# vdBerg93/cl-rrt

Hardware: AMD Instinct MI355X
Metric: nodes expanded/sec (200-obstacle scene) (higher is better)
Workload: dtype f64

## Files before the change

### cl-rrt_amd/clrrt/__init__.py

```python
import ctypes as C
import os

import numpy as np

from . import abi
from .abi import (CLRRT_COLLISION_OBB, CLRRT_COLLISION_OCC, CLRRT_COLLISION_STUB, CLRRT_MODE_BATCH,
                  CLRRT_MODE_EXACT, ROLL_NAMES)

PKG_DIR = os.path.dirname(os.path.dirname(os.path.abspath(__file__)))
LIB_PATH = os.environ.get("CLRRT_LIB") or os.path.join(PKG_DIR, "libclrrt.so")
HEADER_PATH = os.path.join(os.path.dirname(PKG_DIR), "include", "clrrt.h")

_lib = None
P = C.POINTER
EXCHANGE_FN = C.CFUNCTYPE(C.c_int32, C.c_void_p, P(abi.ExchangeIO))

_SIGS = {
    "clrrt_abi_version": (C.c_int, []),
    "clrrt_params_default": (C.c_int, [P(abi.Params), C.c_double, P(C.c_double), C.c_double]),
    "clrrt_rng_seed": (None, [P(abi.Rng), C.c_uint32]),
    "clrrt_rng_next": (C.c_int32, [P(abi.Rng)]),
    "clrrt_draw_samples": (C.c_int, [P(abi.Params), P(abi.Rng), C.c_int32, P(abi.Sample)]),
    "clrrt_create": (C.c_int, [P(abi.Params), P(abi.Capacity), C.c_int, P(C.c_void_p)]),
    "clrrt_destroy": (None, [C.c_void_p]),
# ... 574 lines not shown
    def iterations(self):
        n = C.c_int64()
        self._chk(self.L.clrrt_iteration_records(self.h, 0, 0, None, C.byref(n)), "iteration_records")
        arr = (abi.Iteration * max(1, n.value))()
        self._chk(self.L.clrrt_iteration_records(self.h, 0, n.value, arr, C.byref(n)), "iteration_records")
        return {f: np.array([getattr(arr[i], f) for i in range(n.value)], dtype=np.int64)
                for f, _ in abi.Iteration._fields_}

    def round_sizes(self):
        n = C.c_int64()
        self._chk(self.L.clrrt_round_sizes(self.h, None, 0, C.byref(n)), "round_sizes")
        out = np.zeros(max(1, n.value), dtype=np.int64)
        self._chk(self.L.clrrt_round_sizes(self.h, out.ctypes.data_as(P(C.c_int64)), n.value, C.byref(n)), "round_sizes")
        return out[:n.value]

    def walk_audit(self, samples):
        n = len(samples)
        arr = (abi.Sample * n)(*samples)
        out = np.zeros((n, 20), dtype=np.int32)
        self._chk(self.L.clrrt_walk_audit(self.h, arr, n, out.ctypes.data_as(P(C.c_int32))), "walk_audit")
        return out

    WALK_TILE_DTYPE = np.dtype([(f, np.float32) for f in ("pcx", "pcy", "pr", "rcx", "rcy", "rr", "thx", "thy", "thh",
                                                         "apx", "apy", "aph", "cemin", "aopt")] +
                               [("nonfinite", np.int32), ("eroot", np.float32)])
    WALK_FN_IN = {0: 3, 1: 3, 2: 21, 3: 2, 4: 2}
    WALK_FN_OUT = {0: 2, 1: 2, 2: 2, 3: 2, 4: 3}

    def walk_index(self, first=0, count=None, fused=False):
        if count is None:
# ... 57 lines not shown
```

### cl-rrt_amd/csrc/clrrt_capi.hip

```cpp
#include <hip/hip_runtime.h>
#include <math.h>

#include <algorithm>
#include <climits>
#include <array>
#include <chrono>
#include <cmath>
#include <cstdio>
#include <cstdlib>
#include <cstring>
#include <deque>
#include <functional>
#include <optional>
#include <string>
#include <vector>

#include "../../include/clrrt.h"
#include "clrrt_dev.hpp"
#include "clrrt_devmem_hip.hpp"
#include "clrrt_internal.hpp"

static const int kWalkMaxOver = 2048, kWalkMaxChunks = 64;

using namespace clrrt;
// ... 95 lines not shown
  Job* jobs = nullptr;
  int64_t* totals = nullptr;
  bool totals_zeroed = false;
  unsigned long long* work_ctr = nullptr;
  float* nn_seed = nullptr;
  double bbox[4] = {HUGE_VAL, HUGE_VAL, -HUGE_VAL, -HUGE_VAL};
  double* d_bbox = nullptr;
  double* h_bbox = nullptr;
  int64_t nnw_min_nodes = 8192;
  bool nnw_stateless = false;
  int nnw_bud_tiles = 3072, nnw_bud_ex = 4096, nnw_chunks = 16, nnw_max_over = 1024;
  bool nnw_max_over_set = false;
  bool nnw_bud_tiles_set = false;
  int nnw_half_max = 4096;
  int nnw_hscale = 50;
  int nnw_root_seed = 1;
  int nnw_root_k = 64;
  int nnw_root_scan = 16384;
  int nnw_index = 5;
  int nnw_waves = -1;
  int nnw_double = 1;
  WalkBufs nnw{};
  WalkBufs nnw_alt{};
  BuiltFor nnw_built;
  CompactBufs cmp{};
  int roll_persistent = 1;
  int nn_debug = 0;
  int roll_blocks = 0;
  int n_cu = 256;
  int* roll_q = nullptr;
// ... 1480 lines not shown
    else if (k == "nn_root_k") c->nnw_root_k = (int)value;
    else c->nnw_root_scan = (int)value;
    c->nnw_built.n = -1;
  }
  else if (k == "nn_walk_index" && value >= 0 && value <= 5) {
    c->nnw_index = (int)value;
    c->nnw_built.n = -1;
    c->nnw.sorted_n = c->nnw_alt.sorted_n = c->nnw3.sorted_n = -1;
  }
  else if (k == "nn_walk_waves" && value >= -1 && value <= 1 << 20) c->nnw_waves = (int)value;
  else if (k == "nn_walk_chunks" && value >= 1 && value <= kWalkMaxChunks) c->nnw_chunks = (int)value;
  else if (k == "nn_walk_max_over" && value >= 1 && value <= kWalkMaxOver) {
    c->nnw_max_over = (int)value;
    c->nnw_max_over_set = true;
  }
  else if (k == "nn_walk_double") c->nnw_double = value != 0;
  else if (k == "nn_lag" && (value == 0 || value == 1 || value == 2)) c->nn_lag = (int)value;
  else if (k == "nn_delta_walk") c->nn_delta_walk = value != 0 ? 1 : 0;
  else if (k == "nn_delta_verify") c->nn_delta_verify = value != 0 ? 1 : 0;
  else if (k == "nn_debug" && value >= 0) c->nn_debug = (int)value;
  else if (k == "fail_at_round" && value >= 0 && value < INT_MAX) c->fail_at_round = (int)value;
  else if (k == "fail_after_exchange" && value >= 0 && value < INT_MAX) c->fail_after_exchange = (int)value;
  else if (k == "fail_in_round" && value >= 0 && value < INT_MAX) c->fail_in_round = (int)value;
  else if (k == "shard_hook_world1") c->sh.hook_world1 = value != 0;
  else if (k == "roll_blocks" && value >= 0 && value < (1 << 20)) c->roll_blocks = (int)value;
  else if (k == "nn_pipeline") c->nn_pipeline = value != 0;
  else if (k == "roll_priority") c->roll_priority = value != 0;
  else if (k == "roll_order_verify") c->roll_order_verify = value != 0;
  else if (k == "roll_coop") c->roll_coop = value != 0;
  else if (k == "roll_spread") c->roll_spread = value != 0;
// ... 69 lines not shown
  const int64_t Mp = c->cap.max_nodes + 1024;
  HIPC(c, c->mem.renew(&w.sorder, c->cap.max_batch));
  HIPC(c, c->mem.renew(&w.keys, 2 * M));
  HIPC(c, c->mem.renew(&w.keys2, 2 * M));
  HIPC(c, c->mem.renew(&w.vals, std::max<int64_t>(M, Mp)));
  HIPC(c, c->mem.renew(&w.vals2, M));
  w.tmp_bytes = walk_sort_bytes((int)M);
  HIPC(c, c->mem.renew_bytes(&w.tmp, std::max<size_t>(w.tmp_bytes, 256)));
  HIPC(c, c->mem.renew(&w.Q, Mp));
  HIPC(c, c->mem.renew(&w.CE, Mp));
  HIPC(c, c->mem.renew(&w.ID, Mp));
  HIPC(c, c->mem.renew(&w.HEAD, Mp));
  HIPC(c, c->mem.renew(&w.trun, walk_tile_count(c->cap.max_nodes) + 1));
  HIPC(c, c->mem.renew(&w.tiles, walk_tile_count(c->cap.max_nodes) + 1));
  HIPC(c, c->mem.renew(&w.supers, walk_super_count(c->cap.max_nodes) + 1));
  HIPC(c, c->mem.renew(&w.ovf_n, 1));
  HIPC(c, c->mem.renew(&w.ovf, kWalkMaxOver));
  HIPC(c, c->mem.renew(&w.wctr, 8 + 2 + 64));
  w.roster = w.wctr + 8;
  HIPC(c, c->mem.renew(&w.pk, (int64_t)kWalkMaxOver * kWalkMaxChunks * 11));
  HIPC(c, c->mem.renew(&w.pi, (int64_t)kWalkMaxOver * kWalkMaxChunks * 11));
  HIPC(c, c->mem.renew(&w.skeys, Mp));
  HIPC(c, c->mem.renew(&w.sids, Mp));
  w.sorted_n = -1;
  w.cap_nodes = c->cap.max_nodes;
  w.cap_batch = (int)c->cap.max_batch;
  HIPC(c, c->mem.renew(&w.P, Mp));
  return CLRRT_OK;
}

static int ensure_walk_set(clrrt_ctx* c, WalkBufs& w) {
  w.bud_tiles = c->nnw_bud_tiles_set || c->nnw_bud_tiles == 0
                    ? c->nnw_bud_tiles
                    : (int)std::max<int64_t>(c->nnw_bud_tiles, c->n_nodes >> 11);
  w.bud_ex = c->nnw_bud_ex > 0 ? (int)std::max<int64_t>(c->nnw_bud_ex, c->n_nodes >> 9) : 0;
  w.max_over = c->nnw_max_over_set || c->n_nodes < (6 << 20) ? c->nnw_max_over : kWalkMaxOver;
  w.nch = c->nnw_chunks;
  w.half_max = c->nnw_half_max;
  w.index_kind = c->nnw_index;
  w.hscale_pct = c->nnw_hscale;
  w.root_seed = c->nnw_root_seed;
  w.root_k = c->nnw_root_k;
  w.root_scan = c->nnw_root_scan;
  w.waves = c->nnw_waves < 0 ? 9 * c->n_cu : c->nnw_waves;
  w.waves_min_batch = c->nnw_waves < 0 ? 4 * w.waves : 0;
  return alloc_walk(c, w);
}
static int ensure_walk(clrrt_ctx* c) { return ensure_walk_set(c, c->nnw); }

static NnSetup nn_setup(clrrt_ctx* c) {
  NnSetup su;
  double& x0 = su.x0; double& y0 = su.y0; double& x1 = su.x1; double& y1 = su.y1;
  sample_region(c->params, x0, y0, x1, y1);
  if (c->bbox[0] <= c->bbox[2]) {
    x0 = std::min(x0, c->bbox[0] - 1.0); y0 = std::min(y0, c->bbox[1] - 1.0);
    x1 = std::max(x1, c->bbox[2] + 1.0); y1 = std::max(y1, c->bbox[3] + 1.0);
// ... 1850 lines not shown
  int rc = ensure_walk(c);
  if (rc != CLRRT_OK) return rc;
  memcpy(cur.h_samples, samples, sizeof(clrrt_sample) * n);
  HIPC(c, hipMemcpyAsync(cur.d_samples, cur.h_samples, sizeof(clrrt_sample) * n, hipMemcpyHostToDevice, c->stream));
  c->nnw_built.n = -1;
  HIPC(c, launch_nn_walk_build(c->stream, c->nn, (int)c->n_nodes, su.fr, su.x0, su.y0, su.x1, su.y1, c->nnw));
  const char* const pre = "clrrt_walk_audit: ";
  Scratch<int> d_out;
  HIPC(c, d_out.alloc(20 * (size_t)n));
  HIPP(c, pre, launch_walk_audit(c->stream, cur.d_samples, n, c->nn, (int)c->n_nodes, c->dp, su.fr, c->nnw, d_out));
  HIPP(c, pre, hipMemcpyAsync(out, d_out, sizeof(int32_t) * 20 * (size_t)n, hipMemcpyDeviceToHost, c->stream));
  HIPP(c, pre, hipStreamSynchronize(c->stream));
  return CLRRT_OK;
}

int clrrt_debug_walk_index(clrrt_ctx* c, int64_t first, int64_t count, int32_t fused, double hdr[9], float* P,
                           float* Q, float* CE, int32_t* ID, int32_t* HEAD, int32_t* trun, void* tiles, void* supers,
                           int32_t* roster) {
  if (!c || !hdr) return CLRRT_EINVAL;
  if (first < 0 || count <= 0 || first > c->n_nodes || count > c->n_nodes - first)
    return fail(c, CLRRT_EINVAL, "debug_walk_index: node range outside the tree");
  pf_reset(c);
  HIPC(c, hipSetDevice(c->device));
  const NnSetup su = nn_setup(c);
  const bool whole = !fused && first == 0 && count == c->n_nodes;
  if (!su.region_ok || c->n_nodes < c->nnw_min_nodes || (!fused && !whole && count < c->nnw_min_nodes))
    return fail(c, CLRRT_ESTATE, "the walk does not serve this tree (too small or no region)");
  int rc = CLRRT_OK;
  WalkBufs* w = nullptr;
  if (fused) {
// ... 63 lines not shown
```

### cl-rrt_amd/csrc/clrrt_internal.hpp

```cpp
#pragma once
#include <hip/hip_runtime.h>
#include <stdint.h>

#include "../../include/clrrt.h"
#include "clrrt_dev.hpp"
#include "clrrt_stdsort.hpp"

namespace clrrt {

#define CLRRT_ROLL_PENDING (-2)

struct RollRes {
  double st[10];
  double costE, costS;
  double bx, by;
  double fx, fy;
  double vback;
  int32_t outcome;
  int32_t nrows;
  int32_t refN;
  int32_t pad;
};

struct WorkCtr {
// ... 144 lines not shown
  int2* trun;
  WalkTile *tiles, *supers;
  int bud_tiles, bud_ex, max_over, nch;
  int half_max = 4096;
  int waves = 0;
  int waves_min_batch = 0;
  int index_kind = 0;
  int hscale_pct = 100;
  int* wctr = nullptr;
  int* roster = nullptr;
  int root_seed = 1;
  int root_k = 64;
  int root_scan = 16384;
  float* seed_out = nullptr;
  hipEvent_t ev_main = nullptr;
  int* ovf_n;
  int4* ovf;
  float* pk;
  int* pi;
  uint64_t* skeys;
  int* sids;
  int64_t sorted_n;
  double sorted_x0, sorted_y0, sorted_scale;
  int sorted_kind;
  int64_t cap_nodes;
  int cap_batch;
};
size_t walk_sort_bytes(int n);
int64_t walk_tile_count(int64_t n);
int64_t walk_super_count(int64_t n);
// ... 190 lines not shown
```

### cl-rrt_amd/csrc/clrrt_nnwalk.hip

```cpp
#include <hip/hip_runtime.h>
#include <climits>
#include <hip/hip_fp16.h>
#include <hipcub/hipcub.hpp>
#include <rocprim/device/device_merge.hpp>
#include <algorithm>
#include <stdint.h>

#include "clrrt_dev.hpp"
#include "clrrt_internal.hpp"

namespace clrrt {

#define CAND_K 10
#define NN_K (CAND_K + 1)
#define WALK_TILE 32
#define WALK_SUPER 32
#define WALK_FMT_STATE 0
#define WALK_FMT_HALF 1
#define WALK_FMT_CODED 2
#ifndef WALK_STAGE1_QUEUE
#define WALK_STAGE1_QUEUE 0
#endif
#ifndef WALK_HALF_SUPER
#define WALK_HALF_SUPER 1
// ... 93 lines not shown
    return;
  }
  uint32_t k = 0xffffffffu;
  if (isfinite(x) && isfinite(y)) {
    const double fx = fmin(fmax((x - x0) * scale, 0.0), 65535.0);
    const double fy = fmin(fmax((y - y0) * scale, 0.0), 65535.0);
    k = w_spread((uint32_t)fx) | (w_spread((uint32_t)fy) << 1);
  }
  keys[i] = ((uint64_t)bin << (64 - WALK_SECTOR_BITS)) | ((uint64_t)k << (32 - WALK_SECTOR_BITS)) |
            (__float_as_uint(nodes[i].costE) >> WALK_SECTOR_BITS);
  vals[i] = i;
}

__global__ void k_walk_skeys(const clrrt_sample* __restrict__ S, int B, double x0, double y0, double scale,
                             uint32_t* __restrict__ keys, int* __restrict__ vals, int* __restrict__ zero1,
                             int* __restrict__ zero8) {
  const int i = blockIdx.x * blockDim.x + threadIdx.x;
  if (zero1 && i == 0) *zero1 = 0;
  if (zero8 && i < 8) zero8[i] = 0;
  if (i >= B) return;
  const double x = S[i].x, y = S[i].y;
  uint32_t k = 0xffffffffu;
  if (isfinite(x) && isfinite(y)) {
    const double fx = fmin(fmax((x - x0) * scale, 0.0), 65535.0);
    const double fy = fmin(fmax((y - y0) * scale, 0.0), 65535.0);
    k = w_spread((uint32_t)fx) | (w_spread((uint32_t)fy) << 1);
  }
  keys[i] = k;
  vals[i] = i;
}

__global__ void k_walk_trun(const int* __restrict__ HEAD, const int* __restrict__ ID, int ntiles,
                            int2* __restrict__ trun) {
// ... 499 lines not shown
  float lim = __builtin_inff();
  float cb0 = -2.f;
  int n2 = 0;
#ifdef CLRRT_WALK_PROFILE
  const bool prof = fr.debug == 2;
#else
  constexpr bool prof = false;
#endif
  uint64_t cyc[4] = {0, 0, 0, 0};
#ifdef CLRRT_WALK_PROFILE
  unsigned long long hist[6] = {0, 0, 0, 0, 0, 0};
#endif
  int hc = -1;
  float kc = 0.f;
  __shared__ int s_root[4];
  int seeded = -1;
  if constexpr (!SPLIT) {
    float kr = -__builtin_inff();
    int rX = -1;
    if (roster && !ex) seeded = walk_root_seed(sx, sy, nodes, roster, p.feas_len, lane, kr, rX, lk, li);
    if (lane == 0) {
      s_root[0] = __float_as_int(kr);
      s_root[1] = rX;
      s_root[2] = seeded;
    }
    __builtin_amdgcn_wave_barrier();
  }
  unsigned long long n_sup = 0, n_tile = 0, n_q = 0, n_ex = 0, n_und = 0, n_sure = 0, n_drop = 0;

  auto refresh = [&]() __attribute__((always_inline)) {
    kth = uni(__shfl(lk, NN_K - 1, 64));
// ... 135 lines not shown
    const int cnt = __popcll(m);
    if (cnt == 0) return;
    if (n2 + cnt > 64) drain_exact(cnt);
    __builtin_amdgcn_wave_barrier();
    if (keep) {
      const int pos = n2 + __popcll(m & ((1ull << lane) - 1));
      s_q2[pos] = j;
      s_b2[pos] = lbt;
    }
    n2 += cnt;
    __builtin_amdgcn_wave_barrier();
  };
  auto drain = [&]() __attribute__((always_inline)) { drain_exact(64); };
  auto prefilter = [&](int id, int hd, float4 pp, float4 qq, float ce) __attribute__((always_inline)) -> bool {
    if (hd == hc && !w_less(kc, id, kth, idk)) return false;
    if constexpr (!SPLIT) {
      if (hd & WALK_ROOT_BIT) {
        if (id <= s_root[1] || !w_less(__int_as_float(s_root[0]), id, kth, idk)) return false;
      }
    }
    const float qx = rsx - pp.x, qy = rsy - pp.y;
    const float d2 = qx * qx + qy * qy;
    float l2 = lim;
    if (!ex) {
      const float R = (kth - ce + 2e-4f) * (1.0f / 0.9999f);
      l2 = R < 0.f ? -1.f : (R + dl) * (R + dl);
    }
    if (!(id >= 0 && ((d2 <= l2) || (l2 != l2)))) return false;
    const float vx = rsx - qq.x, vy = rsy - qq.y;
    const float dot = vx * qq.z + vy * qq.w, vv = vx * vx + vy * vy;
    const bool ang_bad = (vv < fl2) || (dot < -1e-3f) || (dot * dot < c45 * c45 * vv && dot >= 0.f);
// ... 66 lines not shown
    n_und += __popcll(__ballot(la == -__builtin_inff())) + __popcll(__ballot(lb == -__builtin_inff()));
    n_sure += __popcll(__ballot(ua < __builtin_inff())) + __popcll(__ballot(ub < __builtin_inff()));
    const bool ia = ub_insert(ua);
    const bool ib2 = ub_insert(ub);
    if (ia || ib2) refresh();
    enqueue(oka, la, ja);
    enqueue(okb, lb, jb);
#endif
    if (prof) cyc[2] += __builtin_amdgcn_s_memtime() - c0;
  };
  auto hmin = [&](float v) -> float {
#pragma unroll
    for (int o = 16; o > 0; o >>= 1) v = fminf(v, __shfl_xor(v, o, 64));
    return v;
  };
  auto run_out = [&](int tl) -> bool {
    const int2 tr = trun[tl];
    if constexpr (!SPLIT) {
      if (tr.x >= 0 && (tr.x & WALK_ROOT_BIT) && !w_less(__int_as_float(s_root[0]), tr.y, kth, idk)) return true;
    }
    return tr.x >= 0 && tr.x == hc && !w_less(kc, tr.y, kth, idk);
  };
  int qn = 0;
  auto next_q = [&]() __attribute__((always_inline)) -> int {
    while (qn > 0) {
      qn--;
      const int t = uni(s_tq[qn]);
      if (!(uni(s_tb[qn]) > kth)) return t;
    }
    return -1;
  };
  auto visit_queue = [&]() __attribute__((always_inline)) {
    const int t0 = next_q();
    const int t1 = next_q();
    const int t2 = next_q();
    const int t3 = next_q();
// ... 8 lines not shown
  };
  auto visit_supers = [&](int la, int lb2, float Tp, float T, bool first) {
    const uint64_t c0 = prof ? __builtin_amdgcn_s_memtime() : 0;
#if WALK_SPLIT_SHARE
    if constexpr (SPLIT && SHARE) refresh();
#endif
    n_sup += 1 + (lb2 >= 0);
    const int sa = gst(la), sb = lb2 >= 0 ? gst(lb2) : -1;
    const int lo = lane < 32 ? la : lb2;
    const int st = lane < 32 ? sa : sb;
    const int tl = st * WALK_SUPER + (lane & 31);
    float lb = __builtin_inff();
    uint64_t tm;
    if constexpr (STATE) {
      const uint32_t vis = st >= 0 ? s_vis[lo] : 0xffffffffu;
      if (st >= 0 && tl < ntiles && !((vis >> (lane & 31)) & 1u)) {
#if WALK_CHEAP_FIRST
        const WalkTile tt = tiles[tl];
        lb = walk_lb_dist(tt, rsx, rsy, ex, dsR);
        if (!(lb > fminf(T, kth))) lb = walk_lb(tt, rsx, rsy, ex, flen_t, dsR);
#else
        lb = walk_lb(tiles[tl], rsx, rsy, ex, flen_t, dsR);
#endif
        if (run_out(tl)) lb = __builtin_inff();
      }
      const bool take = st >= 0 && lb <= T && !(lb > kth);
      const bool drop = st >= 0 && lb > kth;
      tm = __ballot(take);
      const uint64_t dm = __ballot(drop);
      const float rest = hmin(take || drop || st < 0 ? __builtin_inff() : lb);
      if ((lane & 31) == 0 && st >= 0) {
        const int sh = lane;
        s_vis[lo] = vis | (uint32_t)(tm >> sh) | (uint32_t)(dm >> sh);
        s_lbf[lo] = rest;
      }
    } else {
      float slb;
      if constexpr (FMT == WALK_FMT_HALF && WALK_HALF_SUPER) {
        slb = st >= 0 ? __half2float(s_sh[lo]) : __builtin_inff();
// ... 30 lines not shown
    __builtin_amdgcn_wave_barrier();
    while (qn >= 4) visit_queue();
    if (prof) cyc[1] += __builtin_amdgcn_s_memtime() - c0;
  };

  const uint64_t ct0 = prof ? __builtin_amdgcn_s_memtime() : 0;
  auto flush_stats = [&]() {
    if (stats && lane == 0) {
      atomicAdd(&stats[0], n_sup);
      atomicAdd(&stats[1], n_tile);
      atomicAdd(&stats[2], n_q);
      atomicAdd(&stats[3], n_ex);
      atomicAdd(&stats[10], n_und);
      atomicAdd(&stats[11], n_sure);
      atomicAdd(&stats[12], n_drop);
      if (prof) {
        atomicAdd(&stats[4], (unsigned long long)cyc[0]);
        atomicAdd(&stats[5], (unsigned long long)cyc[1]);
        atomicAdd(&stats[6], (unsigned long long)cyc[2]);
        atomicAdd(&stats[7], (unsigned long long)cyc[3]);
        atomicAdd(&stats[8], (unsigned long long)(__builtin_amdgcn_s_memtime() - ct0));
#ifdef CLRRT_WALK_PROFILE
        atomicAdd(&stats[13], hist[0]);
        for (int q = 1; q < 6; q++) atomicAdd(&stats[14 + q], hist[q]);
#endif
      }
    }
  };
  if (SPLIT) refresh();
  if constexpr (!SPLIT) {
// ... 25 lines not shown
  __builtin_amdgcn_wave_barrier();
  if (prof) cyc[0] += __builtin_amdgcn_s_memtime() - ct0;
#ifndef WALK_T0
#define WALK_T0 0.5f
#endif
#ifndef WALK_GROW
#define WALK_GROW 2.f
#endif
  float T = base + WALK_T0, Tp = -__builtin_inff();
#if CLRRT_DELTA_ONEPASS
  if constexpr (SPLIT && !SHARE) {
    if (kb < __builtin_inff()) T = __builtin_inff();
  }
#endif
  bool budget = !SPLIT && (bud_tiles > 0 || bud_ex > 0);
  for (int pass = 0;; pass++) {
    const float lim_t = fminf(T, kth);
    const int lim_c = CODED ? uni(lc_le(lim_t - base)) : 0;
    for (int t0 = 0; t0 < nloc; t0 += 64) {
      const int t = t0 + lane;
      bool want;
      if constexpr (CODED) {
        const int c = t < nloc ? s_lb[t] : 255;
        want = c != 255 && c <= lim_c;
      } else {
        const float lb = t < nloc ? (STATE ? s_lbf[t] : __half2float(s_lbh[t])) : __builtin_inff();
        want = lb < __builtin_inff() && lb <= lim_t;
      }
      uint64_t m = __ballot(want);
      while (m) {
        int sa = -1, sb = -1;
        while (m && sb < 0) {
          const int st = t0 + __ffsll((unsigned long long)m) - 1;
          m &= m - 1;
          if (CODED ? (int)s_lb[st] > kth_c : (STATE ? s_lbf[st] : __half2float(s_lbh[st])) > kth) continue;
          if (sa < 0) sa = st; else sb = st;
        }
        if (sa >= 0) visit_supers(sa, sb, Tp, T, pass == 0);
        if (budget && ((bud_tiles > 0 && n_tile > (unsigned long long)bud_tiles) ||
                       (bud_ex > 0 && n_ex > (unsigned long long)bud_ex))) {
          int slot = 0;
          if (lane == 0) slot = atomicAdd(ovf_n, 1);
          slot = uni(__shfl(slot, 0, 64));
          if (slot < max_over) {
            if (lane == 0)
              ovf[slot] = make_int4(s, __float_as_int(kth), idk == 0x7fffffff ? idk : idk + 1,
                                    kth > 0.f ? __float_as_int(kth) : kth == 0.f ? 0 : 0x7f800000);
            if (stats && lane == 0) atomicAdd(&stats[14], 1ull);
            flush_stats();
            return;
          }
          budget = false;
        }
      }
    }
    flush_queue();
    drain();
    if (T == __builtin_inff() || kth <= T) break;
    Tp = T;
    T = base + (T - base) * WALK_GROW;
    if (T > 1e7f) T = __builtin_inff();
  }
  if constexpr (SPLIT) {
    const int o = o_sp;
    if (lane < NN_K) {
      pk[((size_t)o * nch + ch) * NN_K + lane] = lk;
      pi[((size_t)o * nch + ch) * NN_K + lane] = li;
    }
// ... 17 lines not shown
                                                    const WalkTile* __restrict__ tiles, int ntiles,
                                                    const WalkTile* __restrict__ sup, int nsup, DevParams p,
                                                    NnFrame fr, int* __restrict__ cand, float* __restrict__ ckey,
                                                    int* __restrict__ ncand, int* __restrict__ ctie,
                                                    const int* __restrict__ sorder,
                                                    unsigned long long* __restrict__ stats, int bud_tiles,
                                                    int bud_ex, int* __restrict__ ovf_n, int4* __restrict__ ovf,
                                                    int max_over, int nch, float* __restrict__ pk,
                                                    int* __restrict__ pi, int nloc_max, int* __restrict__ wctr,
                                                    const int* __restrict__ roster) {
  if constexpr (SPLIT) {
    const int o = (int)blockIdx.x / nch;
    const int ch = (int)blockIdx.x % nch;
    if (o >= min(*ovf_n, max_over)) return;
    const int4 rec = ovf[o];
    const int nloc = ch < nsup ? (nsup - ch + nch - 1) / nch : 0;
    walk_one<FMT, SPLIT, BRK>(S, B, nodes, P, Q, CE, ID, HEAD, trun, tiles, ntiles, sup, nsup, p, fr, cand, ckey, ncand, ctie, sorder, stats, bud_tiles, bud_ex, ovf_n, ovf, max_over, nch, pk, pi, nloc_max, rec.x, ch, nloc, __int_as_float(rec.y), rec.z, o);
  } else {
    const int per = (B + 7) >> 3;
    const int x0 = (int)(blockIdx.x & 7);
    if constexpr (!PERS) {
      const int t = x0 * per + (int)(blockIdx.x >> 3);
      if (t >= B) return;
      walk_one<FMT, SPLIT, BRK>(S, B, nodes, P, Q, CE, ID, HEAD, trun, tiles, ntiles, sup, nsup, p, fr, cand, ckey, ncand,
                                ctie, sorder, stats, bud_tiles, bud_ex, ovf_n, ovf, max_over, nch, pk, pi, nloc_max,
                                sorder[t], 0, nsup, __builtin_inff(), 0x7fffffff, 0, roster);
      return;
    }
    int k = 0;
    for (;;) {
      int t = -1;
      while (k < 8) {
        const int x = (x0 + k) & 7;
        int i = 0;
        if (threadIdx.x == 0) i = atomicAdd(&wctr[x], 1);
        i = __shfl(i, 0, 64);
        if (i < per && x * per + i < B) { t = x * per + i; break; }
        k++;
      }
      if (t < 0) break;
      walk_one<FMT, SPLIT, BRK>(S, B, nodes, P, Q, CE, ID, HEAD, trun, tiles, ntiles, sup, nsup, p, fr, cand, ckey, ncand, ctie, sorder, stats, bud_tiles, bud_ex, ovf_n, ovf, max_over, nch, pk, pi, nloc_max, sorder[t], 0, nsup, __builtin_inff(), 0x7fffffff, 0, roster);
      __builtin_amdgcn_wave_barrier();
    }
  }
}

__global__ void __launch_bounds__(64) k_walk_merge(const int* __restrict__ ovf_n, const int4* __restrict__ ovf,
                                                   int max_over, int nch, const float* __restrict__ pk,
                                                   const int* __restrict__ pi, int sort_limit, int* __restrict__ cand,
                                                   float* __restrict__ ckey, int* __restrict__ ncand,
                                                   int* __restrict__ ctie) {
  const int o = blockIdx.x;
  if (o >= min(*ovf_n, max_over)) return;
  const int lane = threadIdx.x;
  const int s = ovf[o].x;
  const int n = nch * NN_K;
  const float* k = pk + (size_t)o * n;
  const int* id = pi + (size_t)o * n;
  float lk = __builtin_inff(), pkey = -__builtin_inff();
  int li = 0x7fffffff, pid = INT_MIN;
  for (int r = 0; r < NN_K; r++) {
    float bk = __builtin_inff();
    int bi = 0x7fffffff;
    for (int j = lane; j < n; j += 64) {
      const float kj = k[j];
      const int ij = id[j];
      if (w_less(pkey, pid, kj, ij) && w_less(kj, ij, bk, bi)) { bk = kj; bi = ij; }
    }
#pragma unroll
    for (int off = 32; off > 0; off >>= 1) {
      const float ok = __shfl_xor(bk, off, 64);
      const int oi = __shfl_xor(bi, off, 64);
      if (w_less(ok, oi, bk, bi)) { bk = ok; bi = oi; }
    }
    if (lane == r) { lk = bk; li = bi; }
    pkey = bk;
    pid = bi;
  }
  walk_emit(lk, li, lane, s, sort_limit, cand, ckey, ncand, ctie);
}

template <bool BRK>
__global__ void __launch_bounds__(64) k_walk_audit(const clrrt_sample* __restrict__ S, int B,
                                                   const NnRec* __restrict__ nodes, const float4* __restrict__ P,
                                                   const float* __restrict__ CE, const int* __restrict__ ID,
                                                   const int* __restrict__ HEAD, const int2* __restrict__ trun,
                                                   const WalkTile* __restrict__ tiles, int ntiles,
                                                   const WalkTile* __restrict__ sup, DevParams p, NnFrame fr,
                                                   int* __restrict__ out) {
  const int s = blockIdx.x, lane = threadIdx.x;
  if (s >= B) return;
  const double sx = S[s].x, sy = S[s].y;
  const bool ex = S[s].explore != 0;
  float lk = __builtin_inff(), kth = __builtin_inff();
  int li = 0x7fffffff, idk = 0x7fffffff;
  const int Npad = ntiles * WALK_TILE;
  for (int j0 = 0; j0 < Npad; j0 += 64) {
    const int j = j0 + lane;
    const int idj = ID[j];
    float key = __builtin_inff();
    bool c = false;
    if (idj >= 0) {
      const NnRec& r = nodes[idj];
      key = dubins_key(sx, sy, r.x, r.y, r.c, r.s);
      if (!ex) key = r.costE + key;
      c = w_less(key, idj, kth, idk) && feasible_search(sx, sy, r.bx, r.by, r.ca, r.sa, r.ang_par, p.feas_len);
    }
    uint64_t m = __ballot(c);
// ... 87 lines not shown
                                      (j + 1 < Npad && (HEAD[j + 1] & ~WALK_ROOT_BIT) == j));
      n_inrun += __popcll(__ballot(inrun));
    }
  }
#pragma unroll
  for (int o = 32; o > 0; o >>= 1) {
    n_in += __shfl_xor(n_in, o, 64);
    n_unb += __shfl_xor(n_unb, o, 64);
    n_run1 += __shfl_xor(n_run1, o, 64);
    s_pr += __shfl_xor(s_pr, o, 64);
    s_rr += __shfl_xor(s_rr, o, 64);
  }
  if (lane == 0) {
    int* o = out + 20 * (size_t)s;
    o[12] = n_in; o[13] = (int)fminf(s_pr * 1000.f, 2e9f); o[14] = (int)fminf(s_rr * 1000.f, 2e9f); o[15] = n_unb;
    o[16] = n_run1; o[17] = n_inrun; o[18] = 0; o[19] = 0;
    o[0] = n_adm; o[1] = n_use; o[2] = n_le; o[3] = n_s1; o[4] = n_sup; o[5] = ex; o[6] = __float_as_int(kth);
    o[7] = n_rec; o[8] = n_inf; o[9] = n_far; o[10] = n_head; o[11] = n_usele;
  }
}

hipError_t launch_walk_audit(hipStream_t st, const clrrt_sample* S, int B, const NnRec* nodes, int N, const DevParams& p,
                             const NnFrame& fr, const WalkBufs& w, int* out) {
  if (N <= 0 || B <= 0) return hipSuccess;
  const int Npad = (N + WALK_TILE * WALK_SUPER - 1) / (WALK_TILE * WALK_SUPER) * (WALK_TILE * WALK_SUPER);
  const int ntiles = Npad / WALK_TILE, nsup = ntiles / WALK_SUPER;
  if (nsup > w.half_max)
    hipLaunchKernelGGL(k_walk_audit<true>, dim3(B), dim3(64), 0, st, S, B, nodes, w.P, w.CE, w.ID, w.HEAD, w.trun,
                       w.tiles, ntiles, w.supers, p, fr, out);
  else
    hipLaunchKernelGGL(k_walk_audit<false>, dim3(B), dim3(64), 0, st, S, B, nodes, w.P, w.CE, w.ID, w.HEAD, w.trun,
                       w.tiles, ntiles, w.supers, p, fr, out);
  LAUNCH_CHECK3();
  return hipSuccess;
}

int64_t walk_tile_count(int64_t n) {
  const int64_t sz = WALK_TILE * WALK_SUPER;
  return (n + sz - 1) / sz * WALK_SUPER;
}
int64_t walk_super_count(int64_t n) { return walk_tile_count(n) / WALK_SUPER; }

size_t walk_sort_bytes(int n) {
  size_t bytes = 0;
  hipcub::DeviceRadixSort::SortPairs(nullptr, bytes, (const uint64_t*)nullptr, (uint64_t*)nullptr,
                                     (const int*)nullptr, (int*)nullptr, n, 0, 64);
  size_t b2 = 0;
// ... 183 lines not shown
    LAUNCH_CHECK3();
    hipLaunchKernelGGL(k_wscan_fix, dim3(nt), dim3(256), 0, st, w.HEAD, Npad, tmax);
    LAUNCH_CHECK3();
  }
  hipLaunchKernelGGL(k_walk_trun, dim3((ntiles + 255) / 256), dim3(256), 0, st, w.HEAD, w.ID, ntiles, w.trun);
  LAUNCH_CHECK3();
  hipLaunchKernelGGL(k_walk_tiles, dim3(ntiles), dim3(64), 0, st, w.P, w.Q, w.CE, w.ID, ntiles, WALK_TILE,
                     fr.delta, nodes, fr.ox, fr.oy, w.tiles);
  LAUNCH_CHECK3();
  hipLaunchKernelGGL(k_walk_tiles, dim3(nsup), dim3(64), 0, st, w.P, w.Q, w.CE, w.ID, nsup,
                     WALK_TILE * WALK_SUPER, fr.delta, nodes, fr.ox, fr.oy, w.supers);
  LAUNCH_CHECK3();
  return hipSuccess;
}

__device__ __forceinline__ unsigned int w_ord32(float f) {
  const unsigned int b = __float_as_uint(f);
  return (b & 0x80000000u) ? ~b : (b | 0x80000000u);
}
__global__ void k_walk_seed(int B, int limit, const float* __restrict__ ckey, const int* __restrict__ ncand,
                            float* __restrict__ seed) {
  const int s = blockIdx.x * blockDim.x + threadIdx.x;
  if (s >= B) return;
  const float k = (limit > 0 && ncand[s] >= limit) ? ckey[s * CAND_K + limit - 1] : __builtin_inff();
  ((unsigned int*)seed)[s] = w_ord32(k);
}
__global__ void k_walk_seed_ovf(const int* __restrict__ ovf_n, const int4* __restrict__ ovf, int max_over,
                                float* __restrict__ seed) {
  const int o = blockIdx.x * blockDim.x + threadIdx.x;
  if (o >= min(*ovf_n, max_over)) return;
  const int4 rec = ovf[o];
  ((unsigned int*)seed)[rec.x] = w_ord32(__int_as_float(rec.y));
}

// ... 5 lines not shown
  if (N > w.cap_nodes || B > w.cap_batch) return hipErrorInvalidValue;
  const int Npad = (N + WALK_TILE * WALK_SUPER - 1) / (WALK_TILE * WALK_SUPER) * (WALK_TILE * WALK_SUPER);
  const int ntiles = Npad / WALK_TILE, nsup = ntiles / WALK_SUPER;
  const double span = fmax(x1 - x0, y1 - y0);
  const double scale = span > 0 ? 65535.0 / span : 1.0;
  hipError_t e = hipSuccess;
  size_t bytes = 0;
  const int fmt = nsup <= 1280 && !stateless ? WALK_FMT_STATE : (nsup <= w.half_max ? WALK_FMT_HALF : WALK_FMT_CODED);
  const bool brk = fmt == WALK_FMT_CODED;
  const size_t lds = (fmt == WALK_FMT_STATE ? 2 * sizeof(float)
                      : fmt == WALK_FMT_HALF ? (WALK_HALF_SUPER ? 2 : 1) * sizeof(__half)
                                             : 1) *
                     (size_t)nsup;
  const bool pers = w.waves > 0 && w.wctr && B >= w.waves_min_batch;
  const bool split = (w.bud_tiles > 0 || w.bud_ex > 0) && w.max_over > 0 && w.nch > 0 && w.ovf_n;
  hipLaunchKernelGGL(k_walk_skeys, dim3((B + 255) / 256), dim3(256), 0, st, S, B, x0, y0, scale, w.keys, w.vals,
                     split ? w.ovf_n : nullptr, pers ? w.wctr : nullptr);
  LAUNCH_CHECK3();
  bytes = w.tmp_bytes;
  e = hipcub::DeviceRadixSort::SortPairs(w.tmp, bytes, w.keys, w.keys2, w.vals, w.sorder, B, 0, 32, st);
  if (e != hipSuccess) return e;
  const int* sorder = w.sorder;
  const int bt = split ? w.bud_tiles : 0, be = split ? w.bud_ex : 0;
  const int grid = pers ? std::min(((B + 7) >> 3) * 8, std::max(8, w.waves & ~7)) : ((B + 7) >> 3) * 8;
  int* wctr = pers ? w.wctr : nullptr;
  auto run = [&](auto F, auto BK, auto PS) -> hipError_t {
    auto* kfn = &k_walk_search<decltype(F)::value, false, decltype(BK)::value, decltype(PS)::value>;
    if (lds > 64 * 1024) {
      const hipError_t ea = hipFuncSetAttribute((const void*)kfn, hipFuncAttributeMaxDynamicSharedMemorySize, (int)lds);
      if (ea != hipSuccess) return ea;
    }
    hipLaunchKernelGGL(kfn, dim3(grid), dim3(64), lds, st, S, B, nodes, w.P, w.Q, w.CE, w.ID, w.HEAD, w.trun, w.tiles,
// ... 18 lines not shown
    }
  }
  if (w.ev_main && (e = hipEventRecord(w.ev_main, st)) != hipSuccess) return e;
  if (split) {
    const int nl = (nsup + w.nch - 1) / w.nch;
    const void* sfn = brk ? (const void*)&k_walk_search<WALK_FMT_STATE, true, true>
                          : (const void*)&k_walk_search<WALK_FMT_STATE, true, false>;
    if (2 * sizeof(float) * (size_t)nl > 64 * 1024) {
      e = hipFuncSetAttribute(sfn, hipFuncAttributeMaxDynamicSharedMemorySize, (int)(2 * sizeof(float) * (size_t)nl));
      if (e != hipSuccess) return e;
    }
#define WALK_SPLIT(BK)                                                                                           \
  hipLaunchKernelGGL((k_walk_search<WALK_FMT_STATE, true, BK>), dim3(w.max_over * w.nch), dim3(64),               \
                     2 * sizeof(float) * (size_t)nl, st, S, B, nodes, w.P, w.Q, w.CE, w.ID, w.HEAD, w.trun, w.tiles, \
                     ntiles, w.supers, nsup, p, fr, cand, ckey, ncand, ctie, sorder, stats, 0, 0, w.ovf_n, w.ovf,  \
                     w.max_over, w.nch, w.pk, w.pi, nl, nullptr, nullptr)
    if (brk) WALK_SPLIT(true);
    else WALK_SPLIT(false);
#undef WALK_SPLIT
    LAUNCH_CHECK3();
    hipLaunchKernelGGL(k_walk_merge, dim3(w.max_over), dim3(64), 0, st, w.ovf_n, w.ovf, w.max_over, w.nch, w.pk, w.pi,
                       p.sort_limit, cand, ckey, ncand, ctie);
    LAUNCH_CHECK3();
  }
  return hipSuccess;
}

__device__ __forceinline__ float w_dec32(unsigned int u) {
  return __uint_as_float((u & 0x80000000u) ? (u & 0x7fffffffu) : ~u);
}
#ifndef CLRRT_DELTA_WAVES
#define CLRRT_DELTA_WAVES 4
#endif
__global__ void __launch_bounds__(64) __attribute__((amdgpu_waves_per_eu(CLRRT_DELTA_WAVES)))
k_walk_delta(const clrrt_sample* __restrict__ S, int B, const NnRec* __restrict__ nodes, const float4* __restrict__ P,
             const float4* __restrict__ Q, const float* __restrict__ CE, const int* __restrict__ ID,
             const int* __restrict__ HEAD, const int2* __restrict__ trun, const WalkTile* __restrict__ tiles, int ntiles,
// ... 53 lines not shown
```

### include/clrrt.h

```cpp
#ifndef CLRRT_H
#define CLRRT_H

#include <stdint.h>

#ifdef __cplusplus
extern "C" {
#endif

#define CLRRT_ABI_VERSION 11

#define CLRRT_OK 0
#define CLRRT_EINVAL (-1)
#define CLRRT_EHIP (-2)
#define CLRRT_ECAPACITY (-3)
#define CLRRT_ESTATE (-4)

#define CLRRT_MODE_EXACT 0
#define CLRRT_MODE_BATCH 1

#define CLRRT_PARENT_PREV (-2)

#define CLRRT_COLLISION_STUB 0
#define CLRRT_COLLISION_OBB 1
#define CLRRT_COLLISION_OCC 2
// ... 279 lines not shown
int clrrt_debug_grid(clrrt_ctx* ctx, int32_t info_i[6], float info_f[3], uint32_t* start, uint16_t* items,
                     uint16_t* mov);

int clrrt_get_counters(clrrt_ctx* ctx, clrrt_counters* out);
int clrrt_reset_counters(clrrt_ctx* ctx);
int clrrt_work_counters(clrrt_ctx* ctx, int64_t out[3]);

int clrrt_kernel_time(clrrt_ctx* ctx, int32_t which, double* ms, int64_t* launches);
int clrrt_enable_timing(clrrt_ctx* ctx, int32_t on);

int clrrt_set_option(clrrt_ctx* ctx, const char* key, int64_t value);
int clrrt_nn_stats(clrrt_ctx* ctx, int64_t out[19]);
int clrrt_search_work(clrrt_ctx* ctx, int64_t out[4]);
int clrrt_search_work_ex(clrrt_ctx* ctx, int64_t out[8]);
int clrrt_walk_audit(clrrt_ctx* ctx, const clrrt_sample* samples, int32_t n, int32_t* out);
int clrrt_debug_walk_index(clrrt_ctx* ctx, int64_t first, int64_t count, int32_t fused, double hdr[9], float* P,
                           float* Q, float* CE, int32_t* ID, int32_t* HEAD, int32_t* trun, void* tiles, void* supers,
                           int32_t* roster);
int clrrt_selftest_walk(clrrt_ctx* ctx, int32_t fn, const float* in, int32_t n, float* out);
int clrrt_round_sizes(clrrt_ctx* ctx, int64_t* out, int64_t cap, int64_t* n);
int clrrt_debug_counters(clrrt_ctx* ctx, int64_t out[64]);
int clrrt_debug_mem_guard(int64_t bytes);
typedef struct clrrt_mem_report {
  int64_t blocks_checked;
  int64_t guard_bytes_checked;
  int64_t violations;
  int64_t first_serial;
  int64_t first_bytes;
  int64_t first_offset;
  int32_t first_side;
// ... 10 lines not shown
```

Baseline: 1.554 million.

## Route root-dominated walk queries early to the split overflow path

Adds an early-divert mode to the nearest-neighbour walk. A query whose sample lies inside the root node's turning-reachable region (early=1), or every budgeted query (early=2), is pushed straight to the chunked overflow/split search instead of walking serially until the budget runs out. The root-seed key is carried in a second overflow slot so the split and merge kernels can apply root pruning and inject the seed candidate, and the merge kernel now writes seed caps. It also adds audit and debug entry points. The risk is extra overflow traffic and merge work if too many queries are diverted.

```diff
diff --git a/cl-rrt_amd/clrrt/__init__.py b/cl-rrt_amd/clrrt/__init__.py
--- a/cl-rrt_amd/clrrt/__init__.py
+++ b/cl-rrt_amd/clrrt/__init__.py
@@ -612,6 +612,15 @@
         self._chk(self.L.clrrt_round_sizes(self.h, out.ctypes.data_as(P(C.c_int64)), n.value, C.byref(n)), "round_sizes")
         return out[:n.value]
 
+    def walk_caps(self, samples):
+        n = len(samples)
+        arr = (abi.Sample * n)(*samples)
+        out = np.zeros(n, dtype=np.float32)
+        fn = self.L.clrrt_debug_walk_caps
+        fn.restype, fn.argtypes = C.c_int, [C.c_void_p, P(abi.Sample), C.c_int32, P(C.c_float)]
+        self._chk(fn(self.h, arr, n, out.ctypes.data_as(P(C.c_float))), "debug_walk_caps")
+        return out
+
     def walk_audit(self, samples):
         n = len(samples)
         arr = (abi.Sample * n)(*samples)
diff --git a/cl-rrt_amd/csrc/clrrt_capi.hip b/cl-rrt_amd/csrc/clrrt_capi.hip
--- a/cl-rrt_amd/csrc/clrrt_capi.hip
+++ b/cl-rrt_amd/csrc/clrrt_capi.hip
@@ -133,6 +133,7 @@
   bool nnw_bud_tiles_set = false;
   int nnw_half_max = 4096;
   int nnw_hscale = 50;
+  int nnw_early = 1;
   int nnw_root_seed = 1;
   int nnw_root_k = 64;
   int nnw_root_scan = 16384;
@@ -1643,6 +1644,7 @@
     c->nnw_max_over = (int)value;
     c->nnw_max_over_set = true;
   }
+  else if (k == "nn_walk_early" && value >= 0 && value <= 2) c->nnw_early = (int)value;
   else if (k == "nn_walk_double") c->nnw_double = value != 0;
   else if (k == "nn_lag" && (value == 0 || value == 1 || value == 2)) c->nn_lag = (int)value;
   else if (k == "nn_delta_walk") c->nn_delta_walk = value != 0 ? 1 : 0;
@@ -1742,8 +1744,8 @@
   HIPC(c, c->mem.renew(&w.trun, walk_tile_count(c->cap.max_nodes) + 1));
   HIPC(c, c->mem.renew(&w.tiles, walk_tile_count(c->cap.max_nodes) + 1));
   HIPC(c, c->mem.renew(&w.supers, walk_super_count(c->cap.max_nodes) + 1));
-  HIPC(c, c->mem.renew(&w.ovf_n, 1));
-  HIPC(c, c->mem.renew(&w.ovf, kWalkMaxOver));
+  HIPC(c, c->mem.renew(&w.ovf_n, 2));
+  HIPC(c, c->mem.renew(&w.ovf, 2 * kWalkMaxOver));
   HIPC(c, c->mem.renew(&w.wctr, 8 + 2 + 64));
   w.roster = w.wctr + 8;
   HIPC(c, c->mem.renew(&w.pk, (int64_t)kWalkMaxOver * kWalkMaxChunks * 11));
@@ -1768,6 +1770,7 @@
   w.index_kind = c->nnw_index;
   w.hscale_pct = c->nnw_hscale;
   w.root_seed = c->nnw_root_seed;
+  w.early = c->nnw_early;
   w.root_k = c->nnw_root_k;
   w.root_scan = c->nnw_root_scan;
   w.waves = c->nnw_waves < 0 ? 9 * c->n_cu : c->nnw_waves;
@@ -3648,6 +3651,38 @@
   return CLRRT_OK;
 }
 
+int clrrt_debug_walk_caps(clrrt_ctx* c, const clrrt_sample* samples, int32_t n, float* out) {
+  if (!c || !samples || !out || n < 0) return CLRRT_EINVAL;
+  pf_reset(c);
+  ListSet& cur = *c->ls[0];
+  if (n > c->cap.max_batch) return fail(c, CLRRT_ECAPACITY, "batch larger than max_batch");
+  HIPC(c, hipSetDevice(c->device));
+  if (n == 0) return CLRRT_OK;
+  const NnSetup su = nn_setup(c);
+  if (!walk_serves(c, su)) return fail(c, CLRRT_ESTATE, "the walk does not serve this tree (too small or no region)");
+  int rc = ensure_walk(c);
+  if (rc != CLRRT_OK) return rc;
+  memcpy(cur.h_samples, samples, sizeof(clrrt_sample) * n);
+  HIPC(c, hipMemcpyAsync(cur.d_samples, cur.h_samples, sizeof(clrrt_sample) * n, hipMemcpyHostToDevice, c->stream));
+  c->nnw_built.n = -1;
+  const char* const pre = "clrrt_debug_walk_caps: ";
+  c->nnw.seed_out = c->nn_seed;
+  const hipError_t e = launch_nn_walk(c->stream, cur.d_samples, n, c->nn, (int)c->n_nodes, c->dp, su.fr, su.x0, su.y0,
+                                      su.x1, su.y1, c->nnw, cur.cand, cur.ckey, cur.ncand, cur.ctie, c->work_ctr + 18,
+                                      c->nnw_stateless);
+  c->nnw.seed_out = nullptr;
+  HIPP(c, pre, e);
+  HIPP(c, pre, hipMemcpyAsync(out, c->nn_seed, sizeof(float) * (size_t)n, hipMemcpyDeviceToHost, c->stream));
+  HIPP(c, pre, hipStreamSynchronize(c->stream));
+  for (int i = 0; i < n; i++) {
+    uint32_t u;
+    memcpy(&u, &out[i], 4);
+    u = (u & 0x80000000u) ? (u & 0x7fffffffu) : ~u;
+    memcpy(&out[i], &u, 4);
+  }
+  return CLRRT_OK;
+}
+
 int clrrt_debug_walk_index(clrrt_ctx* c, int64_t first, int64_t count, int32_t fused, double hdr[9], float* P,
                            float* Q, float* CE, int32_t* ID, int32_t* HEAD, int32_t* trun, void* tiles, void* supers,
                            int32_t* roster) {
diff --git a/cl-rrt_amd/csrc/clrrt_internal.hpp b/cl-rrt_amd/csrc/clrrt_internal.hpp
--- a/cl-rrt_amd/csrc/clrrt_internal.hpp
+++ b/cl-rrt_amd/csrc/clrrt_internal.hpp
@@ -182,6 +182,7 @@
   int root_scan = 16384;
   float* seed_out = nullptr;
   hipEvent_t ev_main = nullptr;
+  int early = 1;
   int* ovf_n;
   int4* ovf;
   float* pk;
diff --git a/cl-rrt_amd/csrc/clrrt_nnwalk.hip b/cl-rrt_amd/csrc/clrrt_nnwalk.hip
--- a/cl-rrt_amd/csrc/clrrt_nnwalk.hip
+++ b/cl-rrt_amd/csrc/clrrt_nnwalk.hip
@@ -131,9 +131,12 @@
 
 __global__ void k_walk_skeys(const clrrt_sample* __restrict__ S, int B, double x0, double y0, double scale,
                              uint32_t* __restrict__ keys, int* __restrict__ vals, int* __restrict__ zero1,
-                             int* __restrict__ zero8) {
+                             int* __restrict__ zero8, int optv) {
   const int i = blockIdx.x * blockDim.x + threadIdx.x;
-  if (zero1 && i == 0) *zero1 = 0;
+  if (zero1 && i == 0) {
+    zero1[0] = 0;
+    zero1[1] = optv;
+  }
   if (zero8 && i < 8) zero8[i] = 0;
   if (i >= B) return;
   const double x = S[i].x, y = S[i].y;
@@ -663,7 +666,17 @@
   int hc = -1;
   float kc = 0.f;
   __shared__ int s_root[4];
+  constexpr bool ROOTED = !SPLIT || SHARE;
   int seeded = -1;
+  if constexpr (SPLIT && SHARE) {
+    if (lane == 0) {
+      const bool sd = ovf[o_sp].z < 0;
+      s_root[0] = sd ? ovf[max_over + o_sp].x : (int)0xff800000;
+      s_root[1] = sd ? roster[1] : -1;
+      s_root[3] = 0;
+    }
+    __builtin_amdgcn_wave_barrier();
+  }
   if constexpr (!SPLIT) {
     float kr = -__builtin_inff();
     int rX = -1;
@@ -829,7 +842,7 @@
   auto drain = [&]() __attribute__((always_inline)) { drain_exact(64); };
   auto prefilter = [&](int id, int hd, float4 pp, float4 qq, float ce) __attribute__((always_inline)) -> bool {
     if (hd == hc && !w_less(kc, id, kth, idk)) return false;
-    if constexpr (!SPLIT) {
+    if constexpr (ROOTED) {
       if (hd & WALK_ROOT_BIT) {
         if (id <= s_root[1] || !w_less(__int_as_float(s_root[0]), id, kth, idk)) return false;
       }
@@ -926,12 +939,12 @@
     for (int o = 16; o > 0; o >>= 1) v = fminf(v, __shfl_xor(v, o, 64));
     return v;
   };
-  auto run_out = [&](int tl) -> bool {
+  auto run_out = [&](int tl) -> int {
     const int2 tr = trun[tl];
-    if constexpr (!SPLIT) {
-      if (tr.x >= 0 && (tr.x & WALK_ROOT_BIT) && !w_less(__int_as_float(s_root[0]), tr.y, kth, idk)) return true;
-    }
-    return tr.x >= 0 && tr.x == hc && !w_less(kc, tr.y, kth, idk);
+    if constexpr (ROOTED) {
+      if (tr.x >= 0 && (tr.x & WALK_ROOT_BIT) && !w_less(__int_as_float(s_root[0]), tr.y, kth, idk)) return 2;
+    }
+    return tr.x >= 0 && tr.x == hc && !w_less(kc, tr.y, kth, idk) ? 1 : 0;
   };
   int qn = 0;
   auto next_q = [&]() __attribute__((always_inline)) -> int {
@@ -970,6 +983,7 @@
     uint64_t tm;
     if constexpr (STATE) {
       const uint32_t vis = st >= 0 ? s_vis[lo] : 0xffffffffu;
+      int ro = 0;
       if (st >= 0 && tl < ntiles && !((vis >> (lane & 31)) & 1u)) {
 #if WALK_CHEAP_FIRST
         const WalkTile tt = tiles[tl];
@@ -978,7 +992,12 @@
 #else
         lb = walk_lb(tiles[tl], rsx, rsy, ex, flen_t, dsR);
 #endif
-        if (run_out(tl)) lb = __builtin_inff();
+        ro = run_out(tl);
+        if (ro) lb = __builtin_inff();
+      }
+      if constexpr (SPLIT && SHARE) {
+        const int nro = __popcll(__ballot(ro == 2));
+        if (nro && lane == 0) s_root[3] += nro;
       }
       const bool take = st >= 0 && lb <= T && !(lb > kth);
       const bool drop = st >= 0 && lb > kth;
@@ -1039,6 +1058,9 @@
       atomicAdd(&stats[10], n_und);
       atomicAdd(&stats[11], n_sure);
       atomicAdd(&stats[12], n_drop);
+      if constexpr (SPLIT && SHARE) {
+        if (!prof && s_root[3] > 0) atomicAdd(&stats[16], (unsigned long long)s_root[3]);
+      }
       if (prof) {
         atomicAdd(&stats[4], (unsigned long long)cyc[0]);
         atomicAdd(&stats[5], (unsigned long long)cyc[1]);
@@ -1094,6 +1116,20 @@
   }
 #endif
   bool budget = !SPLIT && (bud_tiles > 0 || bud_ex > 0);
+  if constexpr (!SPLIT) {
+    const int early = budget && uni(s_root[2]) >= 0 ? uni(ovf_n[1]) : 0;
+    bool fire = early == 2;
+    if (early == 1) {
+      const NnRec& r0 = nodes[0];
+      const float qx = rsx - (float)(r0.x - fr.ox), qy = rsy - (float)(r0.y - fr.oy);
+      const float tx = r0.c * qx - r0.s * qy, ty = fabsf(r0.s * qx + r0.c * qy);
+      fire = uni((int)(tx * tx + ty * (ty - 2.f * rho) < 0.f)) != 0;
+    }
+    if (fire) {
+      if (lane == 0) s_root[2] |= 512;
+      __builtin_amdgcn_wave_barrier();
+    }
+  }
   for (int pass = 0;; pass++) {
     const float lim_t = fminf(T, kth);
     const int lim_c = CODED ? uni(lc_le(lim_t - base)) : 0;
@@ -1116,22 +1152,30 @@
           if (CODED ? (int)s_lb[st] > kth_c : (STATE ? s_lbf[st] : __half2float(s_lbh[st])) > kth) continue;
           if (sa < 0) sa = st; else sb = st;
         }
-        if (sa >= 0) visit_supers(sa, sb, Tp, T, pass == 0);
+        if (sa < 0) continue;
         if (budget && ((bud_tiles > 0 && n_tile > (unsigned long long)bud_tiles) ||
-                       (bud_ex > 0 && n_ex > (unsigned long long)bud_ex))) {
+                       (bud_ex > 0 && n_ex > (unsigned long long)bud_ex) || uni(s_root[2]) >= 512)) {
+          const bool sd = uni(s_root[2]) >= 512;
           int slot = 0;
           if (lane == 0) slot = atomicAdd(ovf_n, 1);
           slot = uni(__shfl(slot, 0, 64));
           if (slot < max_over) {
             if (lane == 0)
-              ovf[slot] = make_int4(s, __float_as_int(kth), idk == 0x7fffffff ? idk : idk + 1,
+              ovf[slot] = make_int4(s, __float_as_int(kth),
+                                    (idk == 0x7fffffff ? idk : idk + 1) | (sd ? (int)0x80000000 : 0),
                                     kth > 0.f ? __float_as_int(kth) : kth == 0.f ? 0 : 0x7f800000);
-            if (stats && lane == 0) atomicAdd(&stats[14], 1ull);
+            if (sd && lane == 0) ovf[max_over + slot].x = s_root[0];
+            if (stats && lane == 0) {
+              atomicAdd(&stats[14], 1ull);
+              if (sd && !prof) atomicAdd(&stats[15], 1ull);
+            }
             flush_stats();
             return;
           }
           budget = false;
+          if (lane == 0) s_root[2] &= ~512;
         }
+        visit_supers(sa, sb, Tp, T, pass == 0);
       }
     }
     flush_queue();
@@ -1179,8 +1223,10 @@
     const int ch = (int)blockIdx.x % nch;
     if (o >= min(*ovf_n, max_over)) return;
     const int4 rec = ovf[o];
+    const int ib0 = rec.z & 0x7fffffff;
+    const float kb0 = __int_as_float(rec.y);
     const int nloc = ch < nsup ? (nsup - ch + nch - 1) / nch : 0;
-    walk_one<FMT, SPLIT, BRK>(S, B, nodes, P, Q, CE, ID, HEAD, trun, tiles, ntiles, sup, nsup, p, fr, cand, ckey, ncand, ctie, sorder, stats, bud_tiles, bud_ex, ovf_n, ovf, max_over, nch, pk, pi, nloc_max, rec.x, ch, nloc, __int_as_float(rec.y), rec.z, o);
+    walk_one<FMT, SPLIT, BRK>(S, B, nodes, P, Q, CE, ID, HEAD, trun, tiles, ntiles, sup, nsup, p, fr, cand, ckey, ncand, ctie, sorder, stats, bud_tiles, bud_ex, ovf_n, ovf, max_over, nch, pk, pi, nloc_max, rec.x, ch, nloc, kb0, ib0, o, roster);
   } else {
     const int per = (B + 7) >> 3;
     const int x0 = (int)(blockIdx.x & 7);
@@ -1210,11 +1256,18 @@
   }
 }
 
+__device__ __forceinline__ unsigned int w_ord32(float f) {
+  const unsigned int b = __float_as_uint(f);
+  return (b & 0x80000000u) ? ~b : (b | 0x80000000u);
+}
 __global__ void __launch_bounds__(64) k_walk_merge(const int* __restrict__ ovf_n, const int4* __restrict__ ovf,
                                                    int max_over, int nch, const float* __restrict__ pk,
                                                    const int* __restrict__ pi, int sort_limit, int* __restrict__ cand,
                                                    float* __restrict__ ckey, int* __restrict__ ncand,
-                                                   int* __restrict__ ctie) {
+                                                   int* __restrict__ ctie, float* __restrict__ seed,
+                                                   const clrrt_sample* __restrict__ S,
+                                                   const NnRec* __restrict__ nodes, const int* __restrict__ roster,
+                                                   double feas_len) {
   const int o = blockIdx.x;
   if (o >= min(*ovf_n, max_over)) return;
   const int lane = threadIdx.x;
@@ -1222,11 +1275,19 @@
   const int n = nch * NN_K;
   const float* k = pk + (size_t)o * n;
   const int* id = pi + (size_t)o * n;
+  float sk = __builtin_inff();
+  int si = 0x7fffffff;
+  if (ovf[o].z < 0 && roster) {
+    float kr = 0.f;
+    int rX = -1;
+    walk_root_seed(S[s].x, S[s].y, nodes, roster, feas_len, lane, kr, rX, sk, si);
+  }
   float lk = __builtin_inff(), pkey = -__builtin_inff();
   int li = 0x7fffffff, pid = INT_MIN;
   for (int r = 0; r < NN_K; r++) {
     float bk = __builtin_inff();
     int bi = 0x7fffffff;
+    if (w_less(pkey, pid, sk, si)) { bk = sk; bi = si; }
     for (int j = lane; j < n; j += 64) {
       const float kj = k[j];
       const int ij = id[j];
@@ -1243,6 +1304,11 @@
     pid = bi;
   }
   walk_emit(lk, li, lane, s, sort_limit, cand, ckey, ncand, ctie);
+  if (seed && sort_limit > 0 && sort_limit <= NN_K) {
+    const float kl = __shfl(lk, sort_limit - 1, 64);
+    const int il = __shfl(li, sort_limit - 1, 64);
+    if (lane == 0 && il != 0x7fffffff && !(kl < 0.f)) atomicMin((unsigned int*)seed + s, w_ord32(kl));
+  }
 }
 
 template <bool BRK>
@@ -1252,11 +1318,31 @@
                                                    const int* __restrict__ HEAD, const int2* __restrict__ trun,
                                                    const WalkTile* __restrict__ tiles, int ntiles,
                                                    const WalkTile* __restrict__ sup, DevParams p, NnFrame fr,
-                                                   int* __restrict__ out) {
+                                                   const int* __restrict__ roster, int* __restrict__ out) {
   const int s = blockIdx.x, lane = threadIdx.x;
   if (s >= B) return;
   const double sx = S[s].x, sy = S[s].y;
   const bool ex = S[s].explore != 0;
+  int a_reach = 0, a_seed = 0;
+  if (roster && !ex) {
+    float skr = 0.f, slk = __builtin_inff();
+    int srX = -1, sli = 0x7fffffff;
+    const int sd = walk_root_seed(sx, sy, nodes, roster, p.feas_len, lane, skr, srX, slk, sli);
+    if (sd >= 0) {
+      const float k11 = uni(__shfl(slk, NN_K - 1, 64));
+      const float rx0 = (float)(sx - fr.ox), ry0 = (float)(sy - fr.oy);
+      const float fl0 = (float)p.feas_len * (1.f - 1e-5f) - 4.f * fr.delta;
+      const float Rx0 = (float)(nodes[0].x - fr.ox), Ry0 = (float)(nodes[0].y - fr.oy);
+      const float ds0 = sqrtf((rx0 - Rx0) * (rx0 - Rx0) + (ry0 - Ry0) * (ry0 - Ry0)) * (1.f - 1e-5f) - 2.f * fr.delta - 1e-4f;
+      for (int t0 = 0; t0 < ntiles / WALK_SUPER; t0 += 64) {
+        const int t = t0 + lane;
+        a_reach += __popcll(__ballot(t < ntiles / WALK_SUPER && !(walk_lb(sup[t], rx0, ry0, false, fl0, ds0) > k11)));
+      }
+      const float qx = rx0 - Rx0, qy = ry0 - Ry0;
+      const float tx = nodes[0].c * qx - nodes[0].s * qy, ty = fabsf(nodes[0].s * qx + nodes[0].c * qy);
+      a_seed = (sd + 1) | (tx * tx + ty * (ty - 2.f * 4.77f) < 0.f ? 256 : 0);
+    }
+  }
   float lk = __builtin_inff(), kth = __builtin_inff();
   int li = 0x7fffffff, idk = 0x7fffffff;
   const int Npad = ntiles * WALK_TILE;
@@ -1374,7 +1460,7 @@
   if (lane == 0) {
     int* o = out + 20 * (size_t)s;
     o[12] = n_in; o[13] = (int)fminf(s_pr * 1000.f, 2e9f); o[14] = (int)fminf(s_rr * 1000.f, 2e9f); o[15] = n_unb;
-    o[16] = n_run1; o[17] = n_inrun; o[18] = 0; o[19] = 0;
+    o[16] = n_run1; o[17] = n_inrun; o[18] = a_reach; o[19] = a_seed;
     o[0] = n_adm; o[1] = n_use; o[2] = n_le; o[3] = n_s1; o[4] = n_sup; o[5] = ex; o[6] = __float_as_int(kth);
     o[7] = n_rec; o[8] = n_inf; o[9] = n_far; o[10] = n_head; o[11] = n_usele;
   }
@@ -1387,10 +1473,10 @@
   const int ntiles = Npad / WALK_TILE, nsup = ntiles / WALK_SUPER;
   if (nsup > w.half_max)
     hipLaunchKernelGGL(k_walk_audit<true>, dim3(B), dim3(64), 0, st, S, B, nodes, w.P, w.CE, w.ID, w.HEAD, w.trun,
-                       w.tiles, ntiles, w.supers, p, fr, out);
+                       w.tiles, ntiles, w.supers, p, fr, (const int*)w.roster, out);
   else
     hipLaunchKernelGGL(k_walk_audit<false>, dim3(B), dim3(64), 0, st, S, B, nodes, w.P, w.CE, w.ID, w.HEAD, w.trun,
-                       w.tiles, ntiles, w.supers, p, fr, out);
+                       w.tiles, ntiles, w.supers, p, fr, (const int*)w.roster, out);
   LAUNCH_CHECK3();
   return hipSuccess;
 }
@@ -1604,10 +1690,6 @@
   return hipSuccess;
 }
 
-__device__ __forceinline__ unsigned int w_ord32(float f) {
-  const unsigned int b = __float_as_uint(f);
-  return (b & 0x80000000u) ? ~b : (b | 0x80000000u);
-}
 __global__ void k_walk_seed(int B, int limit, const float* __restrict__ ckey, const int* __restrict__ ncand,
                             float* __restrict__ seed) {
   const int s = blockIdx.x * blockDim.x + threadIdx.x;
@@ -1643,8 +1725,9 @@
                      (size_t)nsup;
   const bool pers = w.waves > 0 && w.wctr && B >= w.waves_min_batch;
   const bool split = (w.bud_tiles > 0 || w.bud_ex > 0) && w.max_over > 0 && w.nch > 0 && w.ovf_n;
+  const int early = split && w.roster && w.root_seed ? w.early : 0;
   hipLaunchKernelGGL(k_walk_skeys, dim3((B + 255) / 256), dim3(256), 0, st, S, B, x0, y0, scale, w.keys, w.vals,
-                     split ? w.ovf_n : nullptr, pers ? w.wctr : nullptr);
+                     split ? w.ovf_n : nullptr, pers ? w.wctr : nullptr, early);
   LAUNCH_CHECK3();
   bytes = w.tmp_bytes;
   e = hipcub::DeviceRadixSort::SortPairs(w.tmp, bytes, w.keys, w.keys2, w.vals, w.sorder, B, 0, 32, st);
@@ -1693,13 +1776,13 @@
   hipLaunchKernelGGL((k_walk_search<WALK_FMT_STATE, true, BK>), dim3(w.max_over * w.nch), dim3(64),               \
                      2 * sizeof(float) * (size_t)nl, st, S, B, nodes, w.P, w.Q, w.CE, w.ID, w.HEAD, w.trun, w.tiles, \
                      ntiles, w.supers, nsup, p, fr, cand, ckey, ncand, ctie, sorder, stats, 0, 0, w.ovf_n, w.ovf,  \
-                     w.max_over, w.nch, w.pk, w.pi, nl, nullptr, nullptr)
+                     w.max_over, w.nch, w.pk, w.pi, nl, nullptr, (const int*)w.roster)
     if (brk) WALK_SPLIT(true);
     else WALK_SPLIT(false);
 #undef WALK_SPLIT
     LAUNCH_CHECK3();
     hipLaunchKernelGGL(k_walk_merge, dim3(w.max_over), dim3(64), 0, st, w.ovf_n, w.ovf, w.max_over, w.nch, w.pk, w.pi,
-                       p.sort_limit, cand, ckey, ncand, ctie);
+                       p.sort_limit, cand, ckey, ncand, ctie, w.seed_out, S, nodes, (const int*)w.roster, p.feas_len);
     LAUNCH_CHECK3();
   }
   return hipSuccess;
diff --git a/include/clrrt.h b/include/clrrt.h
--- a/include/clrrt.h
+++ b/include/clrrt.h
@@ -317,6 +317,7 @@
 int clrrt_search_work(clrrt_ctx* ctx, int64_t out[4]);
 int clrrt_search_work_ex(clrrt_ctx* ctx, int64_t out[8]);
 int clrrt_walk_audit(clrrt_ctx* ctx, const clrrt_sample* samples, int32_t n, int32_t* out);
+int clrrt_debug_walk_caps(clrrt_ctx* ctx, const clrrt_sample* samples, int32_t n, float* out);
 int clrrt_debug_walk_index(clrrt_ctx* ctx, int64_t first, int64_t count, int32_t fused, double hdr[9], float* P,
                            float* Q, float* CE, int32_t* ID, int32_t* HEAD, int32_t* trun, void* tiles, void* supers,
                            int32_t* roster);
```

Result: slower. 1.520 million (-2.2%).
